# AbbVie-ComputationalGenomics/SAIGEgds

Measured on AMD Instinct MI355X. Metric: variants/sec seqAssocGLMM_SPA at N=430K; achieved HBM GB/s vs roofline, higher is better.
Workload: dtype f64

## Files before the change

saigegds_amd/csrc/dev_common.h:

```cpp
#pragma once
#include "s3_layout.h"

struct RowsRef {
	const uint8_t *base;
	size_t bpv;
	int ntile;
	const unsigned *cptr, *cidx;
	const uint8_t *corient;
};
__device__ __forceinline__ size_t rr_piece(const RowsRef &rr, size_t j, size_t p)
{
	return rr.ntile ? s3_piece_off(j, p, rr.ntile) : j * rr.bpv + p * 16;
}
__device__ __forceinline__ size_t rr_row_bytes(const RowsRef &rr) { return rr.ntile ? (size_t)rr.ntile * 64 : rr.bpv; }
__device__ __forceinline__ const uint8_t *rr_row(const RowsRef &rr, size_t j) { return rr.base + j * rr.bpv; }


struct DevModel {
	int N, K, P, quant;
	double tau0, r;
	double thr_maf, thr_mac, thr_missing, thr_spa;
	const double *F;
	const double *X;
	const double *y;
// ... 247 lines not shown
__device__ __forceinline__ VarHead make_head(const DevModel &md, double AC, int Num)
{
	VarHead h;
	const int N = md.N;
	h.AC = AC; h.Num = Num;
	h.AF = (Num > 0) ? (AC / (2 * Num)) : NAN;
	const double maf = fmin(h.AF, 1 - h.AF);
	h.mac = fmin(AC, 2 * Num - AC);
	const double missing = double(N - Num) / N;
	h.pass = (Num > 0) && (maf > 0) && (maf >= md.thr_maf) && (h.mac >= md.thr_mac) &&
		(missing <= md.thr_missing);
	h.minus = h.AF > 0.5;
	const double imp = 2 * h.AF;
	if (h.minus) { h.lut[0] = 2; h.lut[1] = 1; h.lut[2] = 0; h.lut[3] = 2 - imp; }
	else         { h.lut[0] = 0; h.lut[1] = 1; h.lut[2] = 2; h.lut[3] = imp; }
	return h;
}

#define SPA4_TIER_X 0.45
#define SPA5_NNZ 8192
#define SPA5_EXACT_X 1.2
template <int K>
__device__ __forceinline__ int spa_tier(const DevModel &md, int nnz, double S, double var2, double AC2, const double (&c)[KMAX])
{
	double bmax = 0;
#pragma unroll
	for (int k = 0; k < K; k++) bmax += fabs(c[k]) * md.Xabs[k];
	const double t1 = fabs(S) * sqrt(AC2) / (sqrt(md.r) * var2);
	const double x = 1.5 * t1 * (2.0 + bmax) / sqrt(AC2);
	if (nnz <= SPA5_NNZ) return (x <= SPA5_EXACT_X) ? 2 : 3;
	return (x <= SPA4_TIER_X) ? 0 : 1;
}

template <int K>
__device__ __forceinline__ void spa_push(const DevModel &md, SpaRec *recs, int *counters, int btop, int *fb_series,
	int *fb_exact, int j, int minus, double AC2, int nnz, const double (&lut)[4], double pn, double S, double var2,
	const double (&c)[KMAX])
{
	const int tier = btop > 0 ? spa_tier<K>(md, nnz, S, var2, AC2, c) : 0;
	int slot;
	if (tier >= 2) {
		slot = btop + atomicAdd(&counters[5], 1);
		if (tier == 2) fb_series[atomicAdd(&counters[3], 1)] = slot;
		else fb_exact[atomicAdd(&counters[4], 1)] = slot;
	} else {
		slot = tier ? btop - 1 - atomicAdd(&counters[7], 1) : atomicAdd(&counters[0], 1);
	}
	SpaRec *r = recs + slot;
	r->j = j; r->minus = minus; r->nnz = nnz; r->has_gmu = 0;
#pragma unroll
	for (int k = 0; k < 4; k++) r->lut[k] = lut[k];
	r->AC2 = AC2; r->p_noadj = pn; r->S = S; r->var2 = var2; r->sum_gmu = 0;
	r->tscale = spa_tscale(S, var2, AC2, md.r);
#pragma unroll
	for (int k = 0; k < KMAX; k++) r->c[k] = c[k];
}

template <int K>
__device__ __forceinline__ int score_epilogue(const DevModel &md, const VarHead &h, const double (&acc)[2 * K + 2],
	double *out, double (&c_out)[KMAX], double *p_noadj_out, double *S_out, double *var2_out)
{
	const double s = acc[2 * K], w = acc[2 * K + 1];
	double quad = 0, ec = 0, sac = 0;
#pragma unroll
	for (int a = 0; a < K; a++) {
		const double ca = acc[a];
#pragma unroll
		for (int b = 0; b < K; b++) quad += ca * acc[b] * md.XVX[a * K + b];
		ec += acc[K + a] * ca;
		sac += md.S_a[a] * ca;
	}
	const double var2 = quad + w - 2 * ec;
	const double S = s - sac;
	double pval, beta;
	if (md.quant) {
		const double inv_sqrt_mac = 1.0 / sqrt(h.mac), inv_mac = 1.0 / h.mac;
		const double var1 = var2 * inv_mac * md.r;
// ... 49 lines not shown
```

saigegds_amd/csrc/host_init.h:

```cpp
extern "C" const char *sgx_version(void) { return "saigehip 0.1 (gfx950)"; }
extern "C" const char *sgx_last_error(void) { return g_err.c_str(); }

extern "C" int sgx_device_count(void)
{
	int n = 0;
	if (hipGetDeviceCount(&n) != hipSuccess) return 0;
	return n;
}

extern "C" size_t sgx_row_stride(int32_t n_samp)
{
	return (size_t)((n_samp + 511) / 512) * 128;
}

static double thr_or(double v, double dflt) { return std::isfinite(v) ? v : dflt; }

extern "C" int sgx_set_thresholds(sgx_handle *h, double maf, double mac, double missing,
	double spa_pval)
{
	if (!h) return fail(SGX_EINVAL, "sgx_set_thresholds: NULL handle");
	h->md.thr_maf = thr_or(maf, -1);
	h->md.thr_mac = thr_or(mac, -1);
	h->md.thr_missing = thr_or(missing, 1);
	h->md.thr_spa = thr_or(spa_pval, 0.05);
// ... 324 lines not shown
		if (h->pin_valid[b]) (void)hipHostFree(h->pin_valid[b]);
	}
	(void)hipFree(h->pipe_flag);
	if (h->h_pipe_flag) (void)hipHostFree(h->h_pipe_flag);
	if (h->ev_h2d) (void)hipEventDestroy(h->ev_h2d);
	for (int k = 0; k < 2; k++) { if (h->ev_copy[k]) (void)hipEventDestroy(h->ev_copy[k]); if (h->ev_done[k]) (void)hipEventDestroy(h->ev_done[k]); }
	if (h->cstream) (void)hipStreamDestroy(h->cstream);
	(void)hipFree(h->stage_in); (void)hipFree(h->stage_out); (void)hipFree(h->stage_valid); (void)hipFree(h->stage_pk); (void)hipFree(h->ds_part);
	if (h->h_counters) (void)hipHostFree(h->h_counters);
	for (int i = 0; i < 3; i++) if (h->ev[i]) (void)hipEventDestroy(h->ev[i]);
	for (int i = 0; i < 2; i++) if (h->evk[i]) (void)hipEventDestroy(h->evk[i]);
	if (h->ev_lists) (void)hipEventDestroy(h->ev_lists);
	if (h->s3_side) { (void)hipStreamSynchronize(h->s3_side); (void)hipStreamDestroy(h->s3_side); }
	if (h->hstream) { (void)hipStreamSynchronize(h->hstream); (void)hipStreamDestroy(h->hstream); }
	if (h->s3_fork) (void)hipEventDestroy(h->s3_fork);
	if (h->s3_join) (void)hipEventDestroy(h->s3_join);
	if (h->stream) (void)hipStreamDestroy(h->stream);
	delete h;
}

static int ensure_recs(sgx_handle *h, size_t n)
{
	if (n <= h->recs_cap) return SGX_OK;
	HIPCHK(hipStreamSynchronize(h->stream));
	if (h->recs) HIPCHK(hipFree(h->recs));
	if (h->fallback) HIPCHK(hipFree(h->fallback));
	h->recs = nullptr; h->fallback = nullptr; h->recs_cap = 0;
	HIPCHK(hipMalloc((void **)&h->recs, 3 * n * sizeof(SpaRec)));
	HIPCHK(hipMalloc((void **)&h->fallback, n * sizeof(int)));
	if (!h->md.quant) {
		if (h->fb_spa2) HIPCHK(hipFree(h->fb_spa2));
		h->fb_spa2 = nullptr;
		h->nseg = (h->md.N + spa_seg(h->md.K) - 1) / spa_seg(h->md.K);
		HIPCHK(hipMalloc((void **)&h->fb_spa2, n * sizeof(int)));
		if (h->fb_x2) HIPCHK(hipFree(h->fb_x2));
		h->fb_x2 = nullptr;
		HIPCHK(hipMalloc((void **)&h->fb_x2, n * sizeof(int)));
		if (h->seg4) HIPCHK(hipFree(h->seg4));
		h->seg4 = nullptr;
		h->vcap4 = (int)std::min<size_t>(n, 65536);
		h->nround4 = (int)((n + h->vcap4 - 1) / h->vcap4);
		HIPCHK(hipMalloc((void **)&h->seg4, (size_t)h->nseg * SPA4_NSMAX * h->vcap4 * sizeof(double)));
	}
	if (h->mf_ok) {
		if (h->mf_acc) HIPCHK(hipFree(h->mf_acc));
		h->mf_acc = nullptr;
		HIPCHK(hipMalloc((void **)&h->mf_acc, n * (size_t)(2 * h->mfe.acc_stride - 16) * sizeof(int)));
	}
	h->recs_cap = n;
	return SGX_OK;
}
```

saigegds_amd/csrc/host_lanes.h:

```cpp
extern "C" int sgx_set_option(sgx_handle *h, const char *name, long long value)
{
	if (!h || !name) return fail(SGX_EINVAL, "sgx_set_option: NULL argument");
	const std::string n(name);
	if (n == "score_v1") h->force_v1 = value != 0;
	else if (n == "force_dense") h->force_dense = value != 0;
	else if (n == "spa_exact") h->force_exact = value != 0;
	else if (n == "pipe_mb") { if (value < 0 || value > 65536) return fail(SGX_EINVAL, "pipe_mb out of range"); h->pipe_bytes = (size_t)value << 20; return SGX_OK; }
	else if (n == "spa_abl") h->spa_abl = (int)value;
	else if (n == "guard_exp") { if (value < 0 || value > 300) return fail(SGX_EINVAL, "guard_exp must be 0..300"); h->guard_tol = std::pow(10.0, -(double)value); }
	else if (n == "three_plane") { if (value < -1 || value > 1) return fail(SGX_EINVAL, "three_plane must be -1 (automatic), 0 or 1"); h->dense_opt = (int)value; return SGX_OK; }
	else if (n == "lanes") {
		if (value < 1 || value > 4) return fail(SGX_EINVAL, "lanes must be 1..4");
		if (h->owner) return fail(SGX_EINVAL, "lanes: not on a twin");
		int rc = sgx_sync(h);
		if (rc) return rc;
		for (int i = (int)value - 1; i < 3; i++) if (h->twins[i]) { sgx_free(h->twins[i]); h->twins[i] = nullptr; }
		for (int i = 0; i < (int)value - 1; i++) {
			if (h->twins[i]) continue;
			sgx_handle *t = new sgx_handle();
			t->device = h->device; t->md = h->md; t->mf_ok = h->mf_ok; t->mfe = h->mfe;
			for (int g = 0; g < MF_MAXG; g++) { t->mf[g] = h->mf[g]; t->mf_nbfv[g] = h->mf_nbfv[g]; }
			t->dF = h->dF; t->dX = h->dX; t->dy = h->dy; t->dmu = h->dmu; t->dmu2 = h->dmu2; t->dXM = h->dXM; t->dFl = h->dFl; t->dQ = h->dQ;
			t->shares_model = true; t->owner = h;
			t->force_dense = h->force_dense; t->force_v1 = h->force_v1; t->force_exact = h->force_exact;
// ... 20 lines not shown
	into.score_launches += x.score_launches; into.spa_launches += x.spa_launches;
	into.three_plane += x.three_plane; into.n_unlisted += x.n_unlisted; into.n_guarded += x.n_guarded;
}

static int sync_lane(sgx_handle *h)
{
	int rc = set_dev(h);
	if (rc) return rc;
	HIPCHK(hipStreamSynchronize(h->stream));
	if (h->pend_dense.active) {
		h->pend_dense.active = false;
		if (h->stats_pending && h->h_counters[2] > 0) {
			rc = launch_pending_dense(h);
			if (rc) return rc;
			HIPCHK(hipStreamSynchronize(h->stream));
		}
	}
	if (h->stats_pending) {
		h->stats.n_spa = (uint64_t)(h->h_counters[0] + h->h_counters[7] - h->h_counters[6] + h->h_counters[5]);
		h->stats.n_valid = (uint64_t)h->h_counters[1];
		h->stats.n_spa_dense = (uint64_t)h->h_counters[2];
		h->stats.n_spa_slow = (uint64_t)h->h_counters[4];
		h->stats.three_plane = h->form == FORM_THREE ? 1u : 0u;
		h->stats.n_guarded = (uint32_t)h->h_counters[21];
		h->stats.n_unlisted = (uint32_t)h->h_counters[23] - h->stats.n_guarded;
		if (h->form != FORM_FP64) {
			sgx_handle *p = h->owner ? h->owner : h;
			const double frac = 64.0 * (double)h->h_counters[22] / ((double)std::max<uint64_t>(1, h->stats.n_variants) * (double)h->md.N);
			const bool over = (uint64_t)h->stats.n_unlisted * 32 > h->stats.n_variants;
			if (h->form != FORM_THREE && (frac > SGX_DENSE_ON || over)) p->dense_mode = true;
			else if (h->form == FORM_THREE && frac < SGX_DENSE_OFF) p->dense_mode = false;
		}
#ifdef SPA5_PROF
		fprintf(stderr, "routing: tier A %d, tier B %d (of them handed on by A: %d), per-variant kernels %d (series list %d, exact list %d), dense %d\n",
			h->h_counters[0], h->h_counters[7], h->h_counters[6], h->h_counters[5], h->h_counters[3], h->h_counters[4], h->h_counters[2]);
		fprintf(stderr, "spa5 phases (10 ns ticks summed over variants): series kernel %d variants: stage %d count %d index %d gather %d series %d (sweep %d sum %d solve %d) | exact kernel %d variants: stage %d count %d index %d gather %d - sweeps %d\n",
			h->h_counters[3], h->h_counters[8], h->h_counters[9], h->h_counters[10], h->h_counters[11], h->h_counters[12], h->h_counters[13], h->h_counters[14], h->h_counters[15],
			h->h_counters[4], h->h_counters[16], h->h_counters[17], h->h_counters[18], h->h_counters[19], h->h_counters[21]);
#endif
		float a = 0, b = 0, c = 0;
		(void)hipEventElapsedTime(&a, h->ev[0], h->ev[1]);
		(void)hipEventElapsedTime(&b, h->ev[1], h->ev[2]);
		(void)hipEventElapsedTime(&c, h->ev[0], h->ev[2]);
		h->stats.ms_score = a; h->stats.ms_spa = b; h->stats.ms_total = c;
		float k = 0;
		if (h->evk_set) (void)hipEventElapsedTime(&k, h->evk[0], h->evk[1]);
		h->stats.ms_kernel = k; h->evk_set = false;
		float l = 0;
		if (h->lists_timed) { (void)hipEventElapsedTime(&l, h->ev_lists, h->ev[0]); h->stats.ms_total += l; }
		h->stats.ms_lists = l; h->lists_timed = false;
		h->stats_pending = false;
		sgx_handle *p = h->owner ? h->owner : h;
		stats_add(p->total, h->stats);
		p->total_calls++;
	}
	return SGX_OK;
}

extern "C" int sgx_sync(sgx_handle *h)
{
	if (!h) return fail(SGX_EINVAL, "sgx_sync: NULL handle");
	int rc = sync_lane(h);
	for (sgx_handle *t : h->twins) if (!rc && t) rc = sync_lane(t);
	return rc;
}

extern "C" int sgx_get_stats(sgx_handle *h, sgx_stats *st)
{
	if (!h || !st) return fail(SGX_EINVAL, "sgx_get_stats: NULL argument");
	int rc = sgx_sync(h);
	if (rc) return rc;
// ... 15 lines not shown
```

saigegds_amd/csrc/host_spa.h:

```cpp


template <int LO, typename F, int... I>
static bool with_int(int v, F &&f, std::integer_sequence<int, I...>)
{
	return ((v == LO + I && (f(std::integral_constant<int, LO + I>()), true)) || ...);
}
template <typename F>
static bool with_k(int K, F &&f) { return with_int<1>(K, f, std::make_integer_sequence<int, KMAX>()); }
template <typename F>
static void with_pp(int P, F &&f)
{
	if (P <= 8) f(std::integral_constant<int, 8>());
	else if (P <= 16) f(std::integral_constant<int, 16>());
	else if (P <= 32) f(std::integral_constant<int, 32>());
	else f(std::integral_constant<int, 64>());
}

static dim3 mf_grid(int n_cu, size_t rows, int ntile, int *tps, int vpb = MF_VPB, int wg_per_cu = 2)
{
	const int vt = (int)((rows + vpb - 1) / vpb);
	int sk = std::max(1, (n_cu * wg_per_cu * 4 + vt / 2) / vt);
	sk = std::min(sk, std::max(1, ntile / 24));
	if (sk >= 6) sk = (sk + 7) & ~7;
	sk = std::min(sk, std::max(1, ntile / 2));
// ... 2 lines not shown
	sk = (ntile + *tps - 1) / *tps;
	return dim3((unsigned)vt, (unsigned)sk);
}

template <int KK, int NCX, int INPUT>
static const void *spa4_moments_fn()
{
	if constexpr (INPUT == IN_2BIT) return (const void *)spa4_moments<KK, NCX>;
	else return (const void *)spa4_moments_ds<KK, NCX, INPUT>;
}

template <int KK, int INPUT>
static int launch_spa_k(sgx_handle *h, RowsRef rr, size_t M, double *out8, bool lazy_dense)
{
	const DevModel &md = h->md;
	constexpr int PB = 512;
	hipStream_t st = h->stream;
	const dim3 sgrid((unsigned)std::min<size_t>(M, (size_t)h->spa_grid));
	if (h->force_v1 && INPUT != IN_2BIT) {
		hipLaunchKernelGGL((spa_kernel<KK, PB, INPUT>), sgrid, dim3(PB), 0, st, rr,
			md, h->recs, h->counters, 0, (const int *)nullptr, h->scratch, h->scratch_stride, out8);
		return SGX_OK;
	}
	const size_t fl = spa4_lds_bytes(KK);
	if (!h->mom_attr_set[INPUT]) {
		HIPCHK(hipFuncSetAttribute(spa4_moments_fn<KK, SPA4_NCA, INPUT>(), hipFuncAttributeMaxDynamicSharedMemorySize, (int)fl));
		HIPCHK(hipFuncSetAttribute(spa4_moments_fn<KK, SPA4_NCB, INPUT>(), hipFuncAttributeMaxDynamicSharedMemorySize, (int)fl));
		h->mom_attr_set[INPUT] = true;
	}
	const int nround = (int)((M + h->vcap4 - 1) / h->vcap4);
	const int btop = (int)(2 * M);
	const dim3 gsolve((unsigned)std::min((h->vcap4 + 3) / 4, 4 * h->n_cu));
	const size_t rowb5 = (size_t)((md.N + 63) / 64) * 16;
	const size_t l5 = (INPUT == IN_2BIT && rowb5 <= 120 * 1024) ? rowb5 : 0;
	const bool small5 = INPUT == IN_2BIT && rowb5 <= 32 * 1024;
	if (l5 > 48 * 1024 && !h->spa5_attr_set[INPUT]) {
		HIPCHK(hipFuncSetAttribute((const void *)spa5_kernel<KK, INPUT, 0, 512>, hipFuncAttributeMaxDynamicSharedMemorySize, (int)l5));
		HIPCHK(hipFuncSetAttribute((const void *)spa5_kernel<KK, INPUT, 1, 512>, hipFuncAttributeMaxDynamicSharedMemorySize, (int)l5));
		h->spa5_attr_set[INPUT] = true;
	}
	const int fx5 = (h->force_exact ? 1 : 0) | (h->spa_abl & ~1);
	auto moments = [&](auto ncx, int tier, int rd) {
		constexpr int NCX = decltype(ncx)::value;
		if constexpr (INPUT == IN_2BIT)
			hipLaunchKernelGGL((spa4_moments<KK, NCX>), dim3((unsigned)h->n_cu), dim3(WAVE * spa4_waves(KK)), fl, st, rr, md, h->nseg,
				tier, btop, rd * h->vcap4, h->vcap4, h->recs, h->counters, h->seg4, h->spa_abl, h->cur5 + 2);
		else
			hipLaunchKernelGGL((spa4_moments_ds<KK, NCX, INPUT>), dim3((unsigned)h->n_cu), dim3(WAVE * spa4_waves(KK)), fl, st,
				(const void *)rr.base, rr.bpv, md, h->nseg, tier, btop, rd * h->vcap4, h->vcap4, h->recs, h->counters, h->seg4, h->cur5 + 2);
		hipLaunchKernelGGL((spa4_solve<KK, NCX>), gsolve, dim3(256), 0, st, md, h->nseg, tier, btop, rd * h->vcap4, h->vcap4,
			h->recs, h->counters, h->seg4, h->fallback, h->fb_x2, out8, h->force_dense ? 1 : 0, h->force_exact ? 1 : 0);
	};
	for (int rd = 0; rd < nround; rd++) moments(std::integral_constant<int, SPA4_NCA>(), 0, rd);
	for (int rd = 0; rd < nround; rd++) moments(std::integral_constant<int, SPA4_NCB>(), 1, rd);
	const int only5 = (INPUT == IN_2BIT && rr.cptr != nullptr && (h->spa_abl & 512)) ? 2 : 0;
	const size_t ws5 = spa5_wg_bytes(md.N);
	auto spa5 = [&](auto threads, int nwg) {
		constexpr int T5 = decltype(threads)::value;
		if constexpr (T5 == 512 || INPUT == IN_2BIT) {
			hipLaunchKernelGGL((spa5_kernel<KK, INPUT, 0, T5>), dim3((unsigned)nwg), dim3(T5), l5, st, rr, md, h->recs, h->counters,
				h->fb_spa2, h->fb_x2, h->cur5, h->fallback, h->scr5, out8, h->force_dense ? 1 : 0, fx5, l5, only5, ws5, 3);
			hipLaunchKernelGGL((spa5_kernel<KK, INPUT, 1, T5>), dim3((unsigned)nwg), dim3(T5), l5, st, rr, md, h->recs, h->counters,
				h->fb_x2, h->fb_x2, h->cur5 + 1, h->fallback, h->scr5, out8, h->force_dense ? 1 : 0, fx5, l5, only5, ws5, 4);
		}
	};
	if (small5) spa5(std::integral_constant<int, 128>(), h->nwg5);
	else spa5(std::integral_constant<int, 512>(), h->n_cu);
	if (!lazy_dense)
		hipLaunchKernelGGL((spa_kernel<KK, PB, INPUT>), sgrid, dim3(PB), 0, st, rr,
			md, h->recs, h->counters, 2, h->fallback, h->scratch, h->scratch_stride, out8);
	return SGX_OK;
}

template <int INPUT>
static int launch_spa(sgx_handle *h, RowsRef rr, size_t M, double *out8, bool lazy_dense = false)
{
	h->stats.spa_launches = 0;
	if (h->md.quant) return SGX_OK;
	int rc = SGX_OK;
	with_k(h->md.K, [&](auto kk) { rc = launch_spa_k<decltype(kk)::value, INPUT>(h, rr, M, out8, lazy_dense); });
	if (rc) return rc;
	HIPCHK(hipGetLastError());
	const bool v1 = h->force_v1 && INPUT != IN_2BIT;
	h->stats.spa_launches = v1 ? 1u : (uint32_t)(4 * ((M + h->vcap4 - 1) / h->vcap4) + 3);
	if (lazy_dense && !v1) { h->pend_dense.active = true; h->pend_dense.rr = rr; h->pend_dense.M = M; h->pend_dense.out8 = out8; }
	return SGX_OK;
}

static int launch_pending_dense(sgx_handle *h)
{
	const dim3 sgrid((unsigned)std::min<size_t>(h->pend_dense.M, (size_t)h->spa_grid));
	with_k(h->md.K, [&](auto kk) {
		hipLaunchKernelGGL((spa_kernel<decltype(kk)::value, 512, IN_2BIT>), sgrid, dim3(512), 0, h->stream, h->pend_dense.rr, h->md,
			h->recs, h->counters, 2, h->fallback, h->scratch, h->scratch_stride, h->pend_dense.out8);
	});
	HIPCHK(hipGetLastError());
	return SGX_OK;
}

static int scan_begin(sgx_handle *h, hipStream_t sst, ScanForm form, const sgx_block *b)
{
	h->form = form;
	if (b) HIPCHK(hipStreamWaitEvent(sst, b->ready, 0));
	if (form == FORM_FP64) {
		HIPCHK(hipMemsetAsync(h->counters, 0, 24 * sizeof(int), sst));
		if (h->cur5) HIPCHK(hipMemsetAsync(h->cur5, 0, 8 * sizeof(int), sst));
	}
	HIPCHK(hipEventRecord(h->ev[0], sst));
	return SGX_OK;
}

template <int INPUT>
static int scan_end(sgx_handle *h, hipStream_t sst, const sgx_block *b, RowsRef rr, size_t M, double *out8, bool lazy_dense)
{
	HIPCHK(hipEventRecord(h->ev[1], sst));
	h->stats.score_launches = h->form == FORM_FP64 ? 1 : 5;
	if (sst != h->stream) HIPCHK(hipStreamWaitEvent(h->stream, h->ev[1], 0));
// ... 67 lines not shown
```

saigegds_amd/csrc/kern_spa4.h:

```cpp
#pragma once
#include "kern_spa4_tab.h"


#ifndef SPA4_WAVES_LOWK
#define SPA4_WAVES_LOWK 8
#endif
__host__ __device__ constexpr int spa4_waves(int K) { return K <= 8 ? SPA4_WAVES_LOWK : 8; }
#define SPA4_NCA 12
#define SPA4_NCB SPA4_NC
#define SPA4_NSMAX (SPA4_NC + 5)
#define SPA4_TAIL_TOL 1e-10

__device__ __forceinline__ double spa4_fma_svv(double a_sgpr, double x, double c_vgpr)
{
	double r;
	asm("v_fma_f64 %0, %1, %2, %3" : "=v"(r) : "s"(a_sgpr), "v"(x), "v"(c_vgpr));
	return r;
}

__device__ __forceinline__ void spa4_max_abs(double &g, double a)
{
	asm("v_max_f64 %0, %0, |%1|" : "+v"(g) : "v"(a));
}

// ... 477 lines not shown
	const double sdev = qtilde - m1, qinv = -sdev + m1;
	const double pn_in = d_pchisq1_upper(sdev * sdev / var2);
	if (fabs(qtilde - m1) / sqrt(var2) < 2.0) {
		if (lane == 0) spa_write_row(r, Tstat, var1, pn_in, true, out8);
		return;
	}
	const double nb = (xsum_c - a[1]) * inv;
	const double L = a[2] + fmax(-nb, 0.0), U = a[3] + fmin(-nb, 0.0);
	const double mar = 1e-9 * (fabs(L) + fabs(U) + fabs(qtilde) + fabs(qinv));
	if (force_dense || !(qtilde < L - mar && qtilde > U + mar && qinv < L - mar && qinv > U + mar)) {
		if (lane == 0) fb_dense[atomicAdd(&counters[2], 1)] = ri;
		return;
	}
	Spa4Series<NC> S;
	S.k1 = a[4]; S.k2 = a[5]; S.ts = r.tscale; S.gmax = a[NS - 1];
#pragma unroll
	for (int x = 0; x < NC - 2; x++) S.kp[x] = a[6 + x];
	const double NAmu = m1 - a[4], NAsigma = var2 - a[5];
	const double qmine = lane == 0 ? qtilde : qinv;
	RootState sm;
	const bool ok_mine = !force_exact && spa4_root(S, md.spa_xmax, qmine, NAmu, NAsigma, sm);
	double p_mine = 0;
	if (ok_mine && sm.converged) p_mine = lugannani_rice(sm.root, sm.Kcur, sm.K2cur, qmine, NAmu, NAsigma);
	const int st_mine = (ok_mine ? 1 : 0) | (ok_mine && sm.converged ? 2 : 0);
	const double p_other = __shfl(p_mine, 1, WAVE);
	const int st_other = __shfl(st_mine, 1, WAVE);
	if (lane != 0) return;
	if (!(st_mine & 1) || !(st_other & 1)) {
		if (tier == 0 && !force_exact) {
			const int slot = atomicAdd(&counters[7], 1);
			atomicAdd(&counters[6], 1);
			recs[btop - 1 - slot] = r;
		} else {
			fb_exact[atomicAdd(&counters[4], 1)] = ri;
		}
		return;
	}
	double pval;
	bool converged = true;
	if ((st_mine & 2) && (st_other & 2)) {
		pval = fabs(p_mine) + fabs(p_other);
		if (pval != 0 && pn_in / pval > 1000) pval = pn_in;
	} else {
		pval = pn_in;
		converged = false;
	}
	spa_write_row(r, Tstat, var1, pval, converged, out8);
}


#define SPA5_BIG 2048

__device__ __forceinline__ void cgf_terms_rt(double g, double m, double t, bool with_k, double &k1, double &k2, double &k0)
{
	const double om = 1 - m, mg = m * g, c2 = om * mg * g;
	const double e = fast_exp(-g * t);
	const double d = fma(om, e, m);
	const double rr = isfinite(d) ? fast_rcp(d) : 0.0;
	k1 = fma(mg, rr, k1);
	const double tt = c2 * e * rr * rr;
	if (isfinite(tt)) k2 += tt;
	if (with_k) k0 += cgf_korg_term(g, m, t, d, om);
}

__host__ __device__ inline size_t spa5_wg_bytes(int N) { return (((size_t)N + 63) & ~(size_t)63) * (16 + 4); }

template <int BLOCK>
__device__ __noinline__ void spa5_cum_sweep(const double2 *__restrict__ glist, int nnz, double ts, double *kp_out)
{
	constexpr int NC = SPA4_NCB;
	double kp[NC - 1];
#pragma unroll
	for (int a = 0; a < NC - 1; a++) kp[a] = 0;
	double2 gn = (int)threadIdx.x < nnz ? glist[threadIdx.x] : make_double2(0.0, 0.5);
	for (int k = threadIdx.x; k < nnz; k += BLOCK) {
		const double2 gm = gn;
		if (k + BLOCK < nnz) gn = glist[k + BLOCK];
		const double mui = gm.y;
		spa4_cum_terms<NC>(gm.x * ts, mui * (1 - mui), 1 - 2 * mui, kp);
		kp[NC - 2] = fmax(kp[NC - 2], fabs(gm.x));
	}
#pragma unroll
	for (int a = 0; a < NC - 1; a++) kp_out[a] = kp[a];
}

__device__ __noinline__ int spa5_series_solve(const double *arg, const SpaRec *__restrict__ rec, double *__restrict__ out8)
{
	constexpr int NC = SPA4_NCB;
	Spa4Series<NC> S;
#pragma unroll
	for (int a = 0; a < NC - 2; a++) S.kp[a] = arg[a];
	S.k1 = arg[NC - 2]; S.k2 = arg[NC - 1]; S.ts = arg[NC]; S.gmax = arg[NC + 1];
	const double xmax = arg[NC + 2], qtilde = arg[NC + 3], qinv = arg[NC + 4], NAmu = arg[NC + 5], NAsigma = arg[NC + 6];
	const double pn_in = arg[NC + 7], Tstat = arg[NC + 8], var1 = arg[NC + 9];
	RootState s1, s2;
	if (!spa4_root(S, xmax, qtilde, NAmu, NAsigma, s1) || !spa4_root(S, xmax, qinv, NAmu, NAsigma, s2)) return 0;
	double pval;
	bool converged = true;
	if (s1.converged && s2.converged) {
		const double p1 = lugannani_rice(s1.root, s1.Kcur, s1.K2cur, qtilde, NAmu, NAsigma);
		const double p2 = lugannani_rice(s2.root, s2.Kcur, s2.K2cur, qinv, NAmu, NAsigma);
		pval = fabs(p1) + fabs(p2);
		if (pval != 0 && pn_in / pval > 1000) pval = pn_in;
	} else {
		pval = pn_in;
		converged = false;
	}
	const SpaRec rr = *rec;
	spa_write_row(rr, Tstat, var1, pval, converged, out8);
	return 1;
}

template <int BLOCK>
__device__ __forceinline__ bool spa5_series(const double2 *__restrict__ glist, int nnz, double ts, double xmax,
	double k1, double k2, double qtilde, double qinv, double NAmu, double NAsigma, double pn_in,
	double Tstat, double var1, const SpaRec *__restrict__ rec, double *__restrict__ out8, double *sh, int *sh_flag, int *prof = nullptr)
{
	constexpr int NC = SPA4_NCB;
	double kp[NC - 1];
#ifdef SPA5_PROF
	long long tp_ = wall_clock64();
#define SPA5_TS(ph) do { if (threadIdx.x == 0) { const long long now_ = wall_clock64(); atomicAdd(&prof[ph], (int)(now_ - tp_)); tp_ = now_; } } while (0)
#else
#define SPA5_TS(ph) do { } while (0)
#endif
	spa5_cum_sweep<BLOCK>(glist, nnz, ts, kp);
	SPA5_TS(0);
	constexpr int NWV = BLOCK / WAVE;
	double gmax = kp[NC - 2];
	const int lane = threadIdx.x & (WAVE - 1), wv = threadIdx.x / WAVE;
	double kr[NC - 2];
#pragma unroll
	for (int a = 0; a < NC - 2; a++) kr[a] = kp[a];
	const int idx = wave_reduce_scatter(kr, lane);
#pragma unroll
	for (int o = 32; o > 0; o >>= 1) gmax = fmax(gmax, __shfl_xor(gmax, o, WAVE));
	double *part = sh + NC + 16;
	if (!(lane & 3) && idx < NC - 2) part[idx * NWV + wv] = kr[0];
	if (lane == 1) part[(NC - 2) * NWV + wv] = gmax;
	__syncthreads();
	double *arg = sh;
	if (threadIdx.x < NC - 2) {
		double t = 0;
		for (int w = 0; w < NWV; w++) t += part[threadIdx.x * NWV + w];
		arg[threadIdx.x] = t;
	}
	__syncthreads();
	SPA5_TS(1);
	if (threadIdx.x == 0) {
		for (int w = 0; w < NWV; w++) gmax = fmax(gmax, part[(NC - 2) * NWV + w]);
		arg[NC - 2] = k1; arg[NC - 1] = k2; arg[NC] = ts; arg[NC + 1] = gmax; arg[NC + 2] = xmax;
		arg[NC + 3] = qtilde; arg[NC + 4] = qinv; arg[NC + 5] = NAmu; arg[NC + 6] = NAsigma;
		arg[NC + 7] = pn_in; arg[NC + 8] = Tstat; arg[NC + 9] = var1;
		*sh_flag = spa5_series_solve(arg, rec, out8);
	}
	SPA5_TS(2);
	__syncthreads();
	const bool done = *sh_flag != 0;
	__syncthreads();
	return done;
}

#ifndef SPA5_REG_WAVES
#define SPA5_REG_WAVES 2
#endif
#define SPA5_WAVES_PER_SIMD(BLOCK) ((BLOCK) == 512 ? SPA5_REG_WAVES : ((BLOCK) / 64 + 3) / 4)
#ifdef SPA5_PROF
#define SPA5_T(ph) do { if (tid == 0) { const long long now_ = wall_clock64(); atomicAdd(&counters[8 + 8 * MODE + (ph)], (int)(now_ - tprev_)); tprev_ = now_; } } while (0)
#else
#define SPA5_T(ph) do { } while (0)
#endif
template <int K, int INPUT, int MODE, int BLOCK>
__global__ void __launch_bounds__(BLOCK, SPA5_WAVES_PER_SIMD(BLOCK))
spa5_kernel(RowsRef rr, DevModel md, const SpaRec *__restrict__ recs,
	int *__restrict__ counters, const int *__restrict__ todo, int *__restrict__ todo_next, int *__restrict__ cursor,
	int *__restrict__ fb_dense, uint8_t *__restrict__ scratch, double *__restrict__ out8, int force_dense, int force_exact,
	size_t lds_row_bytes, int only, size_t wg_stride, int nslot)
{
	constexpr int KP = (K + 2) & ~1, NW = BLOCK / WAVE;
	extern __shared__ __attribute__((aligned(16))) uint8_t fill_smem[];
	uint4 *rows_lds = reinterpret_cast<uint4 *>(fill_smem);
	__shared__ double sh[SPA4_NCB * NW + SPA4_NCB + 16];
	__shared__ int sh_flag;
	__shared__ int shi[NW];
	__shared__ int sh_vi, sh_v;
	__shared__ SpaRec sh_rec;
	const int N = md.N, tid = threadIdx.x, lane = tid & (WAVE - 1), wid = tid / WAVE;
	double2 *glist = reinterpret_cast<double2 *>(scratch + (size_t)blockIdx.x * wg_stride);
	uint32_t *ilist = reinterpret_cast<uint32_t *>(glist + (((size_t)N + 63) & ~(size_t)63));
	const int ntodo = counters[nslot];
	const int nvec = INPUT == IN_2BIT ? (int)(min((size_t)((N + 63) >> 6) * 16, rr_row_bytes(rr)) / 16) : (N + 63) >> 6;
	const int per = ((nvec + NW - 1) / NW + WAVE - 1) & ~(WAVE - 1);
	for (;;) {
		__syncthreads();
		if (tid < WAVE) {
			int vi0 = 0;
			if (tid == 0) vi0 = atomicAdd(cursor, 1);
			vi0 = __builtin_amdgcn_readfirstlane(vi0);
			int v0 = -1;
			if (vi0 < 2 * ntodo) {
				v0 = todo[vi0 < ntodo ? vi0 : vi0 - ntodo];
				const double *src = reinterpret_cast<const double *>(recs + v0);
				for (int i = tid; i < (int)(sizeof(SpaRec) / 8); i += WAVE) reinterpret_cast<double *>(&sh_rec)[i] = src[i];
			}
			if (tid == 0) { sh_vi = vi0; sh_v = v0; }
		}
		__syncthreads();
		const int vi = sh_vi;
		if (vi >= 2 * ntodo) break;
#ifdef SPA5_PROF
		long long tprev_ = wall_clock64();
#endif
		const bool big_round = vi < ntodo;
		const int v = sh_v;
		const SpaRec &r = sh_rec;
		if ((r.nnz > SPA5_BIG) != big_round) continue;
		auto row_piece = [&](int p) -> uint4 { return *reinterpret_cast<const uint4 *>(rr.base + rr_piece(rr, (size_t)r.j, (size_t)p)); };
		const uint32_t zx = r.minus ? 0xAAAAAAAAu : 0u;
		const double lut0 = r.lut[0], lut1 = r.lut[1], lut2 = r.lut[2], lut3 = r.lut[3];
		const bool listed = INPUT == IN_2BIT && only != 2 && rr.cptr != nullptr && rr.corient[r.j] == (r.minus ? 2 : 1);
		const uint32_t *il = listed ? rr.cidx + rr.cptr[r.j] : ilist;
		int nnz = listed ? r.nnz : 0;
		if (!listed) {
			const bool staged = INPUT == IN_2BIT && lds_row_bytes >= (size_t)nvec * 16;
			if (staged) {
				constexpr int UN = 8;
				for (int p0 = tid; p0 < nvec; p0 += UN * BLOCK) {
					uint4 t[UN];
	#pragma unroll
					for (int j = 0; j < UN; j++) { const int p = p0 + j * BLOCK; t[j] = p < nvec ? row_piece(p) : make_uint4(0u, 0u, 0u, 0u); }
	#pragma unroll
					for (int j = 0; j < UN; j++) { const int p = p0 + j * BLOCK; if (p < nvec) rows_lds[p] = t[j]; }
				}
				__syncthreads();
			}
			SPA5_T(0);
			auto masks = [&](int p, uint32_t (&ww)[4], uint32_t (&z)[4]) -> int {
				int cnt = 0;
				if (INPUT == IN_2BIT) {
					uint4 w = make_uint4(0u, 0u, 0u, 0u);
					if (p < nvec) w = staged ? rows_lds[p] : row_piece(p);
					ww[0] = w.x; ww[1] = w.y; ww[2] = w.z; ww[3] = w.w;
	#pragma unroll
					for (int k = 0; k < 4; k++) { z[k] = nz_fields((ww[k] ^ zx) & keep_mask(N - p * 64 - 16 * k)); cnt += __popc(z[k]); }
				} else {
					z[0] = z[1] = z[2] = z[3] = 0;
					if (p < nvec) {
						for (int s2 = 0; s2 < 64; s2++) {
							const int i = p * 64 + s2;
							if (i < N && load_dosage<INPUT>(rr, i, r) != 0) { z[s2 >> 5] |= 1u << (s2 & 31); cnt++; }
						}
					}
				}
				return cnt;
			};
			int cnt_w = 0;
			for (int it = 0; it < per; it += WAVE) {
				uint32_t ww[4], z[4];
				cnt_w += masks(wid * per + it + lane, ww, z);
			}
			cnt_w = wave_sum_i(cnt_w);
			if (lane == 0) shi[wid] = cnt_w;
			__syncthreads();
			int o_w = 0;
	#pragma unroll
			for (int w = 0; w < NW; w++) { if (w < wid) o_w += shi[w]; nnz += shi[w]; }
			SPA5_T(1);
			for (int it = 0; it < per; it += WAVE) {
				uint32_t ww[4], z[4];
				const int p = wid * per + it + lane;
				const int cnt = masks(p, ww, z);
				if (!__ballot(cnt != 0)) continue;
				int incl = cnt;
	#pragma unroll
				for (int o = 1; o < WAVE; o <<= 1) {
					const int up = __shfl_up(incl, o, WAVE);
					if (lane >= o) incl += up;
				}
				int o2 = o_w + incl - cnt;
				o_w += __shfl(incl, WAVE - 1, WAVE);
				if (INPUT == IN_2BIT) {
	#pragma unroll
					for (int k = 0; k < 4; k++) {
						uint32_t zz = z[k];
						while (zz) {
							const int b = __ffs(zz) - 1;
							zz &= zz - 1;
							ilist[o2++] = (uint32_t)(p * 64 + 16 * k + (b >> 1)) | (((ww[k] >> b) & 3u) << 30);
						}
					}
				} else {
	#pragma unroll
					for (int k = 0; k < 2; k++) {
						uint32_t zz = z[k];
						while (zz) {
							const int b = __ffs(zz) - 1;
							zz &= zz - 1;
							ilist[o2++] = (uint32_t)(p * 64 + 32 * k + b);
						}
					}
				}
			}
			__syncthreads();
			SPA5_T(2);
		}
		const double inv = 1 / sqrt(r.AC2);
		double c[K];
#pragma unroll
		for (int a = 0; a < K; a++) c[a] = r.c[a];
		double a6[6] = {0, 0, 0, 0, 0, 0};
		constexpr int UNG = K <= 4 ? 4 : 2;
		for (int k0 = tid; k0 < ((force_exact & 128) ? 0 : nnz); k0 += UNG * BLOCK) {
			uint32_t e[UNG];
			double xv[UNG][KP];
#pragma unroll
			for (int j = 0; j < UNG; j++) e[j] = (k0 + j * BLOCK < nnz) ? il[k0 + j * BLOCK] : 0u;
#pragma unroll
			for (int j = 0; j < UNG; j++) {
				const double *x = md.XM + (size_t)(e[j] & 0x3FFFFFFFu) * KP;
#pragma unroll
				for (int a = 0; a < KP; a += 2) {
					const double2 t2 = *reinterpret_cast<const double2 *>(x + a);
					xv[j][a] = t2.x; xv[j][a + 1] = t2.y;
				}
			}
#pragma unroll
			for (int j = 0; j < UNG; j++) {
				const int k = k0 + j * BLOCK;
				if (k >= nnz) continue;
				const uint32_t code = e[j] >> 30;
				const double G = INPUT == IN_2BIT ? ((code & 2u) ? ((code & 1u) ? lut3 : lut2) : ((code & 1u) ? lut1 : lut0))
					: load_dosage<INPUT>(rr, (int)(e[j] & 0x3FFFFFFFu), r);
				double b = 0;
#pragma unroll
				for (int a = 0; a < K; a++) b = fma(xv[j][a], c[a], b);
				const double mui = xv[j][K];
				const double adj = (G - b) * inv;
				glist[k] = make_double2(adj, mui);
				a6[0] = fma(mui, G, a6[0]);
				a6[1] += b;
				if (adj > 0) a6[2] += adj; else a6[3] += adj;
				a6[4] = fma(adj, mui, a6[4]);
				a6[5] = fma(adj * adj, mui * (1 - mui), a6[5]);
			}
		}
		block_sum<6, BLOCK>(a6, sh);
		SPA5_T(3);
		double xmu_c = 0, xsum_c = 0;
#pragma unroll
		for (int a = 0; a < K; a++) { xmu_c = fma(md.Xmu[a], c[a], xmu_c); xsum_c = fma(md.Xsum[a], c[a], xsum_c); }
		const double m1 = (a6[0] - xmu_c) * inv;
		const double Tstat = r.S * inv;
		const double var2 = r.var2 / r.AC2, var1 = var2 * md.r;
		const double qtilde = Tstat / sqrt(var1) * sqrt(var2) + m1;
		const double sdev = qtilde - m1, qinv = -sdev + m1;
		const double pn_in = d_pchisq1_upper(sdev * sdev / var2);
		double pval;
		bool converged = true;
		if (fabs(qtilde - m1) / sqrt(var2) < 2.0) {
			pval = pn_in;
		} else {
			const double nb = (xsum_c - a6[1]) * inv;
			const double L = a6[2] + fmax(-nb, 0.0), U = a6[3] + fmin(-nb, 0.0);
			const double mar = 1e-9 * (fabs(L) + fabs(U) + fabs(qtilde) + fabs(qinv));
			if (force_dense || !(qtilde < L - mar && qtilde > U + mar && qinv < L - mar && qinv > U + mar)) {
				if (tid == 0) fb_dense[atomicAdd(&counters[2], 1)] = v;
				continue;
			}
			const double NAmu = m1 - a6[4], NAsigma = var2 - a6[5];
			if (MODE == 0) {
				if ((force_exact & 1) || !spa5_series<BLOCK>(glist, nnz, r.tscale, md.spa_xmax, a6[4], a6[5], qtilde, qinv, NAmu, NAsigma,
						pn_in, Tstat, var1, &sh_rec, out8, sh, &sh_flag, counters + 13)) {
					if (tid == 0) todo_next[atomicAdd(&counters[4], 1)] = v;
				}
				SPA5_T(4);
				continue;
			}
			RootState s1, s2;
			root_begin(s1, qtilde, L, U);
			root_begin(s2, qinv, L, U);
			root_feed(s1, a6[4], a6[5], NAmu, NAsigma, 0.0, true);
			root_feed(s2, a6[4], a6[5], NAmu, NAsigma, 0.0, true);
			auto sweep = [&](bool a1, bool a2, bool k1w, bool k2w, double t1, double t2, double (&sv)[6]) {
#pragma unroll
				for (int a = 0; a < 6; a++) sv[a] = 0;
				double2 gn = tid < nnz ? glist[tid] : make_double2(0.0, 0.5);
				for (int k0 = tid; k0 < nnz; k0 += BLOCK) {
					const double2 gm = gn;
					if (k0 + BLOCK < nnz) gn = glist[k0 + BLOCK];
					if (a1) cgf_terms_rt(gm.x, gm.y, t1, k1w, sv[0], sv[1], sv[2]);
					if (a2) cgf_terms_rt(gm.x, gm.y, t2, k2w, sv[3], sv[4], sv[5]);
				}
				block_sum<6, BLOCK>(sv, sh);
			};
			while ((s1.active || s2.active) && !(force_exact & 64)) {
				const bool a1 = s1.active, a2 = s2.active, k1w = s1.want_k, k2w = s2.want_k;
				double sv[6];
				sweep(a1, a2, k1w, k2w, s1.tnew, s2.tnew, sv);
				if (a1) root_feed(s1, sv[0], sv[1], NAmu, NAsigma, sv[2], k1w);
				if (a2) root_feed(s2, sv[3], sv[4], NAmu, NAsigma, sv[5], k2w);
			}
			if (s1.converged && s2.converged) {
				if (!(s1.k_ok && s2.k_ok)) {
					double sv[6];
					sweep(!s1.k_ok, !s2.k_ok, true, true, s1.root, s2.root, sv);
					if (!s1.k_ok) s1.Kcur = sv[2];
					if (!s2.k_ok) s2.Kcur = sv[5];
				}
				const double p1 = lugannani_rice(s1.root, s1.Kcur, s1.K2cur, qtilde, NAmu, NAsigma);
				const double p2 = lugannani_rice(s2.root, s2.Kcur, s2.K2cur, qinv, NAmu, NAsigma);
				pval = fabs(p1) + fabs(p2);
				if (pval != 0 && pn_in / pval > 1000) pval = pn_in;
			} else {
				pval = pn_in;
				converged = false;
			}
		}
		if (tid == 0) spa_write_row(r, Tstat, var1, pval, converged, out8);
		SPA5_T(5);
	}
}
```

Before: 17.56 million.

## Merge SPA5 series/exact kernels into one launch with big/small queues and LDS staging

Replaces the two spa5 kernel launches (series mode, then exact mode fed by a second todo list) with a single kernel. Variants are routed at push time into four queues split by list type and by nnz above or below a threshold, with large entries processed first. When a variant fails the series path it falls straight through to the exact root solve in the same workgroup instead of being re-queued and regathered. The index list and the (adj, mu) gather list are placed in LDS when they fit, which removes global scratch round-trips but enlarges the dynamic shared-memory allocation and may lower occupancy.

```diff
diff --git a/saigegds_amd/csrc/dev_common.h b/saigegds_amd/csrc/dev_common.h
--- a/saigegds_amd/csrc/dev_common.h
+++ b/saigegds_amd/csrc/dev_common.h
@@ -303,6 +303,14 @@
 	return (x <= SPA4_TIER_X) ? 0 : 1;
 }
 
+#define SPA5_BIG 2048
+__device__ __forceinline__ void spa5_append(int *__restrict__ counters, int btop, int *__restrict__ fb, bool exact, int nnz, int rec)
+{
+	const bool big = nnz > SPA5_BIG;
+	const int pos = atomicAdd(&counters[(exact ? 19 : 17) + (big ? 0 : 1)], 1);
+	fb[(big ? 0 : btop >> 1) + pos] = rec;
+	if (exact) atomicAdd(&counters[4], 1);
+}
 template <int K>
 __device__ __forceinline__ void spa_push(const DevModel &md, SpaRec *recs, int *counters, int btop, int *fb_series,
 	int *fb_exact, int j, int minus, double AC2, int nnz, const double (&lut)[4], double pn, double S, double var2,
@@ -312,8 +320,7 @@
 	int slot;
 	if (tier >= 2) {
 		slot = btop + atomicAdd(&counters[5], 1);
-		if (tier == 2) fb_series[atomicAdd(&counters[3], 1)] = slot;
-		else fb_exact[atomicAdd(&counters[4], 1)] = slot;
+		spa5_append(counters, btop, tier == 2 ? fb_series : fb_exact, tier != 2, nnz, slot);
 	} else {
 		slot = tier ? btop - 1 - atomicAdd(&counters[7], 1) : atomicAdd(&counters[0], 1);
 	}
diff --git a/saigegds_amd/csrc/host_init.h b/saigegds_amd/csrc/host_init.h
--- a/saigegds_amd/csrc/host_init.h
+++ b/saigegds_amd/csrc/host_init.h
@@ -380,10 +380,10 @@
 		if (h->fb_spa2) HIPCHK(hipFree(h->fb_spa2));
 		h->fb_spa2 = nullptr;
 		h->nseg = (h->md.N + spa_seg(h->md.K) - 1) / spa_seg(h->md.K);
-		HIPCHK(hipMalloc((void **)&h->fb_spa2, n * sizeof(int)));
+		HIPCHK(hipMalloc((void **)&h->fb_spa2, 2 * n * sizeof(int)));
 		if (h->fb_x2) HIPCHK(hipFree(h->fb_x2));
 		h->fb_x2 = nullptr;
-		HIPCHK(hipMalloc((void **)&h->fb_x2, n * sizeof(int)));
+		HIPCHK(hipMalloc((void **)&h->fb_x2, 2 * n * sizeof(int)));
 		if (h->seg4) HIPCHK(hipFree(h->seg4));
 		h->seg4 = nullptr;
 		h->vcap4 = (int)std::min<size_t>(n, 65536);
diff --git a/saigegds_amd/csrc/host_lanes.h b/saigegds_amd/csrc/host_lanes.h
--- a/saigegds_amd/csrc/host_lanes.h
+++ b/saigegds_amd/csrc/host_lanes.h
@@ -76,11 +76,15 @@
 			else if (h->form == FORM_THREE && frac < SGX_DENSE_OFF) p->dense_mode = false;
 		}
 #ifdef SPA5_PROF
-		fprintf(stderr, "routing: tier A %d, tier B %d (of them handed on by A: %d), per-variant kernels %d (series list %d, exact list %d), dense %d\n",
-			h->h_counters[0], h->h_counters[7], h->h_counters[6], h->h_counters[5], h->h_counters[3], h->h_counters[4], h->h_counters[2]);
-		fprintf(stderr, "spa5 phases (10 ns ticks summed over variants): series kernel %d variants: stage %d count %d index %d gather %d series %d (sweep %d sum %d solve %d) | exact kernel %d variants: stage %d count %d index %d gather %d - sweeps %d\n",
-			h->h_counters[3], h->h_counters[8], h->h_counters[9], h->h_counters[10], h->h_counters[11], h->h_counters[12], h->h_counters[13], h->h_counters[14], h->h_counters[15],
-			h->h_counters[4], h->h_counters[16], h->h_counters[17], h->h_counters[18], h->h_counters[19], h->h_counters[21]);
+		{
+			const int *c = h->h_counters;
+			const int n_ser = c[17] + c[18], n_x = c[19] + c[20], n_on = c[4] - n_x;
+			fprintf(stderr, "routing: tier A %d, tier B %d (of them handed on by A: %d), per-variant kernel %d (series list %d of them long %d, exact list %d of them long %d), dense %d\n",
+				c[0], c[7], c[6], c[5], n_ser, c[17], n_x, c[19], c[2]);
+			fprintf(stderr, "spa5 paths: series only %d, series then exact %d, exact only %d\n", n_ser - n_on, n_on, n_x);
+			fprintf(stderr, "spa5 phases (10 ns ticks summed over variants): stage %d count %d index %d gather %d series %d (sweep %d sum %d solve %d) exact sweeps %d\n",
+				c[8], c[9], c[10], c[11], c[12], c[14], c[15], c[16], c[13]);
+		}
 #endif
 		float a = 0, b = 0, c = 0;
 		(void)hipEventElapsedTime(&a, h->ev[0], h->ev[1]);
diff --git a/saigegds_amd/csrc/host_spa.h b/saigegds_amd/csrc/host_spa.h
--- a/saigegds_amd/csrc/host_spa.h
+++ b/saigegds_amd/csrc/host_spa.h
@@ -58,11 +58,13 @@
 	const int btop = (int)(2 * M);
 	const dim3 gsolve((unsigned)std::min((h->vcap4 + 3) / 4, 4 * h->n_cu));
 	const size_t rowb5 = (size_t)((md.N + 63) / 64) * 16;
-	const size_t l5 = (INPUT == IN_2BIT && rowb5 <= 120 * 1024) ? rowb5 : 0;
+	const size_t lrow5 = (INPUT == IN_2BIT && rowb5 <= 120 * 1024) ? rowb5 : 0;
 	const bool small5 = INPUT == IN_2BIT && rowb5 <= 32 * 1024;
+	const size_t lg5 = (small5 || lrow5) ? lrow5 : (size_t)112 * 1024;
+	const int li5 = small5 ? 0 : SPA5_NNZ;
+	const size_t l5 = lg5 + (size_t)li5 * sizeof(uint32_t);
 	if (l5 > 48 * 1024 && !h->spa5_attr_set[INPUT]) {
-		HIPCHK(hipFuncSetAttribute((const void *)spa5_kernel<KK, INPUT, 0, 512>, hipFuncAttributeMaxDynamicSharedMemorySize, (int)l5));
-		HIPCHK(hipFuncSetAttribute((const void *)spa5_kernel<KK, INPUT, 1, 512>, hipFuncAttributeMaxDynamicSharedMemorySize, (int)l5));
+		HIPCHK(hipFuncSetAttribute((const void *)spa5_kernel<KK, INPUT, 512>, hipFuncAttributeMaxDynamicSharedMemorySize, (int)l5));
 		h->spa5_attr_set[INPUT] = true;
 	}
 	const int fx5 = (h->force_exact ? 1 : 0) | (h->spa_abl & ~1);
@@ -84,10 +86,8 @@
 	auto spa5 = [&](auto threads, int nwg) {
 		constexpr int T5 = decltype(threads)::value;
 		if constexpr (T5 == 512 || INPUT == IN_2BIT) {
-			hipLaunchKernelGGL((spa5_kernel<KK, INPUT, 0, T5>), dim3((unsigned)nwg), dim3(T5), l5, st, rr, md, h->recs, h->counters,
-				h->fb_spa2, h->fb_x2, h->cur5, h->fallback, h->scr5, out8, h->force_dense ? 1 : 0, fx5, l5, only5, ws5, 3);
-			hipLaunchKernelGGL((spa5_kernel<KK, INPUT, 1, T5>), dim3((unsigned)nwg), dim3(T5), l5, st, rr, md, h->recs, h->counters,
-				h->fb_x2, h->fb_x2, h->cur5 + 1, h->fallback, h->scr5, out8, h->force_dense ? 1 : 0, fx5, l5, only5, ws5, 4);
+			hipLaunchKernelGGL((spa5_kernel<KK, INPUT, T5>), dim3((unsigned)nwg), dim3(T5), l5, st, rr, md, h->recs, h->counters,
+				h->fb_spa2, h->fb_x2, btop, h->cur5, h->fallback, h->scr5, out8, h->force_dense ? 1 : 0, fx5, lrow5, lg5, li5, only5, ws5);
 		}
 	};
 	if (small5) spa5(std::integral_constant<int, 128>(), h->nwg5);
@@ -108,7 +108,7 @@
 	if (rc) return rc;
 	HIPCHK(hipGetLastError());
 	const bool v1 = h->force_v1 && INPUT != IN_2BIT;
-	h->stats.spa_launches = v1 ? 1u : (uint32_t)(4 * ((M + h->vcap4 - 1) / h->vcap4) + 3);
+	h->stats.spa_launches = v1 ? 1u : (uint32_t)(4 * ((M + h->vcap4 - 1) / h->vcap4) + 2);
 	if (lazy_dense && !v1) { h->pend_dense.active = true; h->pend_dense.rr = rr; h->pend_dense.M = M; h->pend_dense.out8 = out8; }
 	return SGX_OK;
 }
diff --git a/saigegds_amd/csrc/kern_spa4.h b/saigegds_amd/csrc/kern_spa4.h
--- a/saigegds_amd/csrc/kern_spa4.h
+++ b/saigegds_amd/csrc/kern_spa4.h
@@ -533,7 +533,7 @@
 			atomicAdd(&counters[6], 1);
 			recs[btop - 1 - slot] = r;
 		} else {
-			fb_exact[atomicAdd(&counters[4], 1)] = ri;
+			spa5_append(counters, btop, fb_exact, true, r.nnz, ri);
 		}
 		return;
 	}
@@ -550,8 +550,6 @@
 }
 
 
-#define SPA5_BIG 2048
-
 __device__ __forceinline__ void cgf_terms_rt(double g, double m, double t, bool with_k, double &k1, double &k2, double &k0)
 {
 	const double om = 1 - m, mg = m * g, c2 = om * mg * g;
@@ -566,17 +564,26 @@
 
 __host__ __device__ inline size_t spa5_wg_bytes(int N) { return (((size_t)N + 63) & ~(size_t)63) * (16 + 4); }
 
+__device__ __forceinline__ double2 spa5_gl(const double2 *gl, bool lds, int k)
+{
+	if (lds) {
+		const __attribute__((address_space(3))) double *p = (const __attribute__((address_space(3))) double *)(gl + k);
+		return make_double2(p[0], p[1]);
+	}
+	return gl[k];
+}
+
 template <int BLOCK>
-__device__ __noinline__ void spa5_cum_sweep(const double2 *__restrict__ glist, int nnz, double ts, double *kp_out)
+__device__ __noinline__ void spa5_cum_sweep(const double2 *__restrict__ glist, bool lds, int nnz, double ts, double *kp_out)
 {
 	constexpr int NC = SPA4_NCB;
 	double kp[NC - 1];
 #pragma unroll
 	for (int a = 0; a < NC - 1; a++) kp[a] = 0;
-	double2 gn = (int)threadIdx.x < nnz ? glist[threadIdx.x] : make_double2(0.0, 0.5);
+	double2 gn = (int)threadIdx.x < nnz ? spa5_gl(glist, lds, threadIdx.x) : make_double2(0.0, 0.5);
 	for (int k = threadIdx.x; k < nnz; k += BLOCK) {
 		const double2 gm = gn;
-		if (k + BLOCK < nnz) gn = glist[k + BLOCK];
+		if (k + BLOCK < nnz) gn = spa5_gl(glist, lds, k + BLOCK);
 		const double mui = gm.y;
 		spa4_cum_terms<NC>(gm.x * ts, mui * (1 - mui), 1 - 2 * mui, kp);
 		kp[NC - 2] = fmax(kp[NC - 2], fabs(gm.x));
@@ -613,7 +620,7 @@
 }
 
 template <int BLOCK>
-__device__ __forceinline__ bool spa5_series(const double2 *__restrict__ glist, int nnz, double ts, double xmax,
+__device__ __forceinline__ bool spa5_series(const double2 *__restrict__ glist, bool lds, int nnz, double ts, double xmax,
 	double k1, double k2, double qtilde, double qinv, double NAmu, double NAsigma, double pn_in,
 	double Tstat, double var1, const SpaRec *__restrict__ rec, double *__restrict__ out8, double *sh, int *sh_flag, int *prof = nullptr)
 {
@@ -625,7 +632,7 @@
 #else
 #define SPA5_TS(ph) do { } while (0)
 #endif
-	spa5_cum_sweep<BLOCK>(glist, nnz, ts, kp);
+	spa5_cum_sweep<BLOCK>(glist, lds, nnz, ts, kp);
 	SPA5_TS(0);
 	constexpr int NWV = BLOCK / WAVE;
 	double gmax = kp[NC - 2];
@@ -667,16 +674,16 @@
 #endif
 #define SPA5_WAVES_PER_SIMD(BLOCK) ((BLOCK) == 512 ? SPA5_REG_WAVES : ((BLOCK) / 64 + 3) / 4)
 #ifdef SPA5_PROF
-#define SPA5_T(ph) do { if (tid == 0) { const long long now_ = wall_clock64(); atomicAdd(&counters[8 + 8 * MODE + (ph)], (int)(now_ - tprev_)); tprev_ = now_; } } while (0)
+#define SPA5_T(ph) do { if (tid == 0) { const long long now_ = wall_clock64(); atomicAdd(&counters[8 + (ph)], (int)(now_ - tprev_)); tprev_ = now_; } } while (0)
 #else
 #define SPA5_T(ph) do { } while (0)
 #endif
-template <int K, int INPUT, int MODE, int BLOCK>
+template <int K, int INPUT, int BLOCK>
 __global__ void __launch_bounds__(BLOCK, SPA5_WAVES_PER_SIMD(BLOCK))
 spa5_kernel(RowsRef rr, DevModel md, const SpaRec *__restrict__ recs,
-	int *__restrict__ counters, const int *__restrict__ todo, int *__restrict__ todo_next, int *__restrict__ cursor,
+	int *__restrict__ counters, const int *__restrict__ fb_series, const int *__restrict__ fb_exact, int btop, int *__restrict__ cursor,
 	int *__restrict__ fb_dense, uint8_t *__restrict__ scratch, double *__restrict__ out8, int force_dense, int force_exact,
-	size_t lds_row_bytes, int only, size_t wg_stride, int nslot)
+	size_t lds_row_bytes, size_t lds_g_bytes, int lds_i_cap, int only, size_t wg_stride)
 {
 	constexpr int KP = (K + 2) & ~1, NW = BLOCK / WAVE;
 	extern __shared__ __attribute__((aligned(16))) uint8_t fill_smem[];
@@ -684,12 +691,15 @@
 	__shared__ double sh[SPA4_NCB * NW + SPA4_NCB + 16];
 	__shared__ int sh_flag;
 	__shared__ int shi[NW];
-	__shared__ int sh_vi, sh_v;
+	__shared__ int sh_vi, sh_v, sh_x;
 	__shared__ SpaRec sh_rec;
 	const int N = md.N, tid = threadIdx.x, lane = tid & (WAVE - 1), wid = tid / WAVE;
 	double2 *glist = reinterpret_cast<double2 *>(scratch + (size_t)blockIdx.x * wg_stride);
 	uint32_t *ilist = reinterpret_cast<uint32_t *>(glist + (((size_t)N + 63) & ~(size_t)63));
-	const int ntodo = counters[nslot];
+	double2 *gl_l = reinterpret_cast<double2 *>(fill_smem);
+	uint32_t *il_l = reinterpret_cast<uint32_t *>(fill_smem + lds_g_bytes);
+	const int nxb = counters[19], nsb = counters[17], nxs = counters[20], nss = counters[18];
+	const int ntodo = nxb + nsb + nxs + nss, half = btop >> 1;
 	const int nvec = INPUT == IN_2BIT ? (int)(min((size_t)((N + 63) >> 6) * 16, rr_row_bytes(rr)) / 16) : (N + 63) >> 6;
 	const int per = ((nvec + NW - 1) / NW + WAVE - 1) & ~(WAVE - 1);
 	for (;;) {
@@ -698,30 +708,33 @@
 			int vi0 = 0;
 			if (tid == 0) vi0 = atomicAdd(cursor, 1);
 			vi0 = __builtin_amdgcn_readfirstlane(vi0);
-			int v0 = -1;
-			if (vi0 < 2 * ntodo) {
-				v0 = todo[vi0 < ntodo ? vi0 : vi0 - ntodo];
+			int v0 = -1, x0 = 0;
+			if (vi0 < ntodo) {
+				int q = vi0;
+				if (q < nxb) { v0 = fb_exact[q]; x0 = 1; }
+				else if ((q -= nxb) < nsb) v0 = fb_series[q];
+				else if ((q -= nsb) < nxs) { v0 = fb_exact[half + q]; x0 = 1; }
+				else v0 = fb_series[half + q - nxs];
 				const double *src = reinterpret_cast<const double *>(recs + v0);
 				for (int i = tid; i < (int)(sizeof(SpaRec) / 8); i += WAVE) reinterpret_cast<double *>(&sh_rec)[i] = src[i];
 			}
-			if (tid == 0) { sh_vi = vi0; sh_v = v0; }
+			if (tid == 0) { sh_vi = vi0; sh_v = v0; sh_x = x0; }
 		}
 		__syncthreads();
-		const int vi = sh_vi;
-		if (vi >= 2 * ntodo) break;
+		if (sh_vi >= ntodo) break;
 #ifdef SPA5_PROF
 		long long tprev_ = wall_clock64();
 #endif
-		const bool big_round = vi < ntodo;
 		const int v = sh_v;
+		const bool from_exact = sh_x != 0;
 		const SpaRec &r = sh_rec;
-		if ((r.nnz > SPA5_BIG) != big_round) continue;
 		auto row_piece = [&](int p) -> uint4 { return *reinterpret_cast<const uint4 *>(rr.base + rr_piece(rr, (size_t)r.j, (size_t)p)); };
 		const uint32_t zx = r.minus ? 0xAAAAAAAAu : 0u;
 		const double lut0 = r.lut[0], lut1 = r.lut[1], lut2 = r.lut[2], lut3 = r.lut[3];
 		const bool listed = INPUT == IN_2BIT && only != 2 && rr.cptr != nullptr && rr.corient[r.j] == (r.minus ? 2 : 1);
 		const uint32_t *il = listed ? rr.cidx + rr.cptr[r.j] : ilist;
 		int nnz = listed ? r.nnz : 0;
+		bool i_lds = false;
 		if (!listed) {
 			const bool staged = INPUT == IN_2BIT && lds_row_bytes >= (size_t)nvec * 16;
 			if (staged) {
@@ -766,6 +779,8 @@
 			int o_w = 0;
 	#pragma unroll
 			for (int w = 0; w < NW; w++) { if (w < wid) o_w += shi[w]; nnz += shi[w]; }
+			i_lds = __builtin_amdgcn_readfirstlane(nnz <= lds_i_cap && !(force_exact & 256) ? 1 : 0) != 0;
+			auto put = [&](int o, uint32_t e) { if (i_lds) il_l[o] = e; else ilist[o] = e; };
 			SPA5_T(1);
 			for (int it = 0; it < per; it += WAVE) {
 				uint32_t ww[4], z[4];
@@ -787,7 +802,7 @@
 						while (zz) {
 							const int b = __ffs(zz) - 1;
 							zz &= zz - 1;
-							ilist[o2++] = (uint32_t)(p * 64 + 16 * k + (b >> 1)) | (((ww[k] >> b) & 3u) << 30);
+							put(o2++, (uint32_t)(p * 64 + 16 * k + (b >> 1)) | (((ww[k] >> b) & 3u) << 30));
 						}
 					}
 				} else {
@@ -797,7 +812,7 @@
 						while (zz) {
 							const int b = __ffs(zz) - 1;
 							zz &= zz - 1;
-							ilist[o2++] = (uint32_t)(p * 64 + 32 * k + b);
+							put(o2++, (uint32_t)(p * 64 + 32 * k + b));
 						}
 					}
 				}
@@ -805,6 +820,8 @@
 			__syncthreads();
 			SPA5_T(2);
 		}
+		const bool g_lds = __builtin_amdgcn_readfirstlane((size_t)nnz * sizeof(double2) <= lds_g_bytes && !(force_exact & 256) ? 1 : 0) != 0;
+		const double2 *gl = g_lds ? gl_l : glist;
 		const double inv = 1 / sqrt(r.AC2);
 		double c[K];
 #pragma unroll
@@ -815,7 +832,7 @@
 			uint32_t e[UNG];
 			double xv[UNG][KP];
 #pragma unroll
-			for (int j = 0; j < UNG; j++) e[j] = (k0 + j * BLOCK < nnz) ? il[k0 + j * BLOCK] : 0u;
+			for (int j = 0; j < UNG; j++) e[j] = (k0 + j * BLOCK < nnz) ? (i_lds ? il_l[k0 + j * BLOCK] : il[k0 + j * BLOCK]) : 0u;
 #pragma unroll
 			for (int j = 0; j < UNG; j++) {
 				const double *x = md.XM + (size_t)(e[j] & 0x3FFFFFFFu) * KP;
@@ -837,7 +854,7 @@
 				for (int a = 0; a < K; a++) b = fma(xv[j][a], c[a], b);
 				const double mui = xv[j][K];
 				const double adj = (G - b) * inv;
-				glist[k] = make_double2(adj, mui);
+				if (g_lds) gl_l[k] = make_double2(adj, mui); else glist[k] = make_double2(adj, mui);
 				a6[0] = fma(mui, G, a6[0]);
 				a6[1] += b;
 				if (adj > 0) a6[2] += adj; else a6[3] += adj;
@@ -869,13 +886,12 @@
 				continue;
 			}
 			const double NAmu = m1 - a6[4], NAsigma = var2 - a6[5];
-			if (MODE == 0) {
-				if ((force_exact & 1) || !spa5_series<BLOCK>(glist, nnz, r.tscale, md.spa_xmax, a6[4], a6[5], qtilde, qinv, NAmu, NAsigma,
-						pn_in, Tstat, var1, &sh_rec, out8, sh, &sh_flag, counters + 13)) {
-					if (tid == 0) todo_next[atomicAdd(&counters[4], 1)] = v;
-				}
+			if (!from_exact) {
+				const bool done = !(force_exact & 1) && spa5_series<BLOCK>(gl, g_lds, nnz, r.tscale, md.spa_xmax, a6[4], a6[5], qtilde, qinv,
+					NAmu, NAsigma, pn_in, Tstat, var1, &sh_rec, out8, sh, &sh_flag, counters + 14);
 				SPA5_T(4);
-				continue;
+				if (done) continue;
+				if (tid == 0) atomicAdd(&counters[4], 1);
 			}
 			RootState s1, s2;
 			root_begin(s1, qtilde, L, U);
@@ -885,10 +901,11 @@
 			auto sweep = [&](bool a1, bool a2, bool k1w, bool k2w, double t1, double t2, double (&sv)[6]) {
 #pragma unroll
 				for (int a = 0; a < 6; a++) sv[a] = 0;
-				double2 gn = tid < nnz ? glist[tid] : make_double2(0.0, 0.5);
+				auto entry = [&](int k) -> double2 { if (g_lds) return gl_l[k]; return glist[k]; };
+				double2 gn = tid < nnz ? entry(tid) : make_double2(0.0, 0.5);
 				for (int k0 = tid; k0 < nnz; k0 += BLOCK) {
 					const double2 gm = gn;
-					if (k0 + BLOCK < nnz) gn = glist[k0 + BLOCK];
+					if (k0 + BLOCK < nnz) gn = entry(k0 + BLOCK);
 					if (a1) cgf_terms_rt(gm.x, gm.y, t1, k1w, sv[0], sv[1], sv[2]);
 					if (a2) cgf_terms_rt(gm.x, gm.y, t2, k2w, sv[3], sv[4], sv[5]);
 				}
```

New measurement: 17.41 million. About the same (-0.8%).
